# TaliMotzkin/GroupNet

Measured on AMD Instinct MI355X. Metric: scenes/sec GroupNet MS-HGNN forward, NBA N=11 B=512, 1/2/4/8 MI355X, higher is better.
Workload: dtype f32; 1 GPU; MS-HGNN forward (c2): affinity + top-k + pairwise + hyper scales [2, 5, 11], N=11 agents, 512 scenes per GPU (global batch 512), fp32 in and out (matrix stages: f16x3 — v_mfma_f32_32x32x16_f16, x = xh + xl (two fp16 parts), three part-products per product (fp32-accurate; operands beyond the fp16 range fall back to bf16x6 inside the launch)), device Philox noise, hipGraph replay on 4 alternating st; global_batch=512, agents=11, parallelism=batch-sharded x1

## Files before the change

groupnet_amd/csrc/gn_common.hpp:

```cpp
#pragma once
#include <hip/hip_runtime.h>
#include <stdint.h>
#include <stdlib.h>

#include "../../include/groupnet_hip.h"

#define GN_WAVE 64

typedef float f32x16 __attribute__((ext_vector_type(16)));
typedef float f32x4 __attribute__((ext_vector_type(4)));

static inline bool gn_aligned16(const void* p) { return (reinterpret_cast<uintptr_t>(p) & 15u) == 0; }

static inline int gn_check_launch() { return hipGetLastError() == hipSuccess ? GN_OK : GN_ERR_LAUNCH; }

#define GN_REQUIRE_PTR(p) \
  do {                    \
    if ((p) == nullptr) return GN_ERR_NULL; \
  } while (0)
#define GN_REQUIRE_ALIGNED(p) \
  do {                        \
    if (!gn_aligned16(p)) return GN_ERR_ALIGN; \
  } while (0)

__device__ __forceinline__ int gn_uniform(int v) { return __builtin_amdgcn_readfirstlane(v); }
template <typename T>
__device__ __forceinline__ T gn_uniform_load(const T* p) {
  return *(const __attribute__((address_space(4))) T*)p;
}

__device__ __forceinline__ float gn_half_sum(float v) {
#pragma unroll
  for (int m = 16; m >= 1; m >>= 1) v += __shfl_xor(v, m, GN_WAVE);
  return v;
}
__device__ __forceinline__ float gn_wave_sum(float v) {
#pragma unroll
  for (int m = 32; m >= 1; m >>= 1) v += __shfl_xor(v, m, GN_WAVE);
  return v;
}
__device__ __forceinline__ float gn_wave_max(float v) {
#pragma unroll
  for (int m = 32; m >= 1; m >>= 1) v = fmaxf(v, __shfl_xor(v, m, GN_WAVE));
  return v;
}

__device__ __forceinline__ float gn_nonmember_sum(int others, float mx) {
  return others > 0 ? (float)others * expf(0.f - mx) : 0.f;
}

template <typename K>
static inline void gn_allow_big_lds(K kernel) {
  static bool done = false;
  if (!done) {
    (void)hipFuncSetAttribute(reinterpret_cast<const void*>(kernel), hipFuncAttributeMaxDynamicSharedMemorySize,
                              160 * 1024);
    done = true;
  }
}

__device__ __forceinline__ void gn_philox_block(unsigned long long blk, unsigned long long seed, uint32_t (&c)[4]) {
  c[0] = (uint32_t)blk;
  c[1] = (uint32_t)(blk >> 32);
  c[2] = 0u;
  c[3] = 0u;
  uint32_t k0 = (uint32_t)seed, k1 = (uint32_t)(seed >> 32);
#pragma unroll
  for (int r = 0; r < 10; ++r) {
    const uint64_t p0 = (uint64_t)0xD2511F53u * c[0];
    const uint64_t p1 = (uint64_t)0xCD9E8D57u * c[2];
    const uint32_t n0 = (uint32_t)(p1 >> 32) ^ c[1] ^ k0;
    const uint32_t n1 = (uint32_t)p1;
    const uint32_t n2 = (uint32_t)(p0 >> 32) ^ c[3] ^ k1;
    const uint32_t n3 = (uint32_t)p0;
    c[0] = n0;
    c[1] = n1;
    c[2] = n2;
    c[3] = n3;
    k0 += 0x9E3779B9u;
    k1 += 0xBB67AE85u;
  }
}
__device__ __forceinline__ float gn_philox_to_uniform(uint32_t x) { return (float)(x >> 8) * 5.9604644775390625e-08f; }
__device__ __forceinline__ float gn_philox_uniform_at(unsigned long long idx, unsigned long long seed) {
  uint32_t c[4];
  gn_philox_block(idx >> 2, seed, c);
  const int l = (int)(idx & 3);
  const uint32_t x = l == 0 ? c[0] : (l == 1 ? c[1] : (l == 2 ? c[2] : c[3]));
  return gn_philox_to_uniform(x);
}

struct GnSwitches {
  bool xcd;
  bool pool_stage;
  bool agg_lines;
  bool agg_hstage;
  bool scatter_pairs;
  int edge_rb2, agg_rb2;
  int mlp2_xs;
  int n2e_rows;
  long long rb2_min_pairs;
};
static inline GnSwitches gn_read_switches() {
  auto tri = [](const char* name) {
    const char* e = getenv(name);
    return e == nullptr ? -1 : (atoi(e) != 0 ? 1 : 0);
  };
  GnSwitches sw{};
  sw.xcd = tri("GN_XCD") != 0;
  sw.pool_stage = tri("GN_POOL_STAGE") != 0;
  sw.agg_lines = tri("GN_AGG_LINES") != 0;
  sw.agg_hstage = tri("GN_AGG_HSTAGE") != 0;
  sw.scatter_pairs = tri("GN_SCATTER_PAIRS") != 0;
  sw.edge_rb2 = tri("GN_EDGE_RB2");
  sw.agg_rb2 = tri("GN_AGG_RB2");
  sw.mlp2_xs = tri("GN_MLP2_XS");
  sw.n2e_rows = tri("GN_N2E_ROWS");
  const char* e = getenv("GN_RB2_MIN_PAIRS");
  sw.rb2_min_pairs = e != nullptr && atoll(e) > 0 ? atoll(e) : 0;
  return sw;
}

static inline void plan_begin(gn_launch_plan_t& p, int n_groups) {
  p = gn_launch_plan_t{};
  p.n_groups = n_groups;
  p.grid[1] = p.grid[2] = 1;
}

#define GN_MAX_SECTIONS 32
struct XcdSections {
  int first[GN_MAX_SECTIONS + 1];
  int n;
  int enabled;
};
__device__ __forceinline__ int gn_xcd_logical(const XcdSections& S, int p) {
  if (!S.enabled) return p;
  const int x = p & 7;
  int slot = p >> 3;
  for (int g = 0; g < S.n; ++g) {
    const int W = S.first[g + 1] - S.first[g];
    const int lo = (int)(((long long)W * x) >> 3), hi = (int)(((long long)W * (x + 1)) >> 3);
    if (slot < hi - lo) return S.first[g] + lo + slot;
    slot -= hi - lo;
  }
  return -1;
}
static inline int gn_xcd_grid(XcdSections& S, bool on) {
  const int total = S.first[S.n];
  S.enabled = (on && S.n <= GN_MAX_SECTIONS && total >= 64) ? 1 : 0;
  if (!S.enabled) return total;
  int worst = 0;
  for (int x = 0; x < 8; ++x) {
    int c = 0;
    for (int g = 0; g < S.n; ++g) {
      const int W = S.first[g + 1] - S.first[g];
      c += (int)(((long long)W * (x + 1)) >> 3) - (int)(((long long)W * x) >> 3);
    }
    worst = c > worst ? c : worst;
  }
  return 8 * worst;
}

__host__ __device__ __forceinline__ int gn_pair_count(int N) { return N * (N + 1) / 2; }
__device__ __forceinline__ int gn_pair_start(int i, int N) { return i * N - (i * (i - 1)) / 2; }
__device__ __forceinline__ int gn_pair_index(int a, int b, int N) {
  const int i = a < b ? a : b, j = a < b ? b : a;
  return gn_pair_start(i, N) + (j - i);
}
__device__ __forceinline__ void gn_pair_decode(int p, int N, int& i, int& j) {
  const float t = (float)(2 * N + 1);
  int r = (int)((t - sqrtf(t * t - 8.f * (float)p)) * 0.5f);
  r = r < 0 ? 0 : (r > N - 1 ? N - 1 : r);
  while (r + 1 < N && gn_pair_start(r + 1, N) <= p) ++r;
  while (r > 0 && gn_pair_start(r, N) > p) --r;
  i = r;
  j = r + (p - gn_pair_start(r, N));
}
```

groupnet_amd/csrc/gn_mlp_bf16.hpp:

```cpp
#pragma once
#include "gn_mlp_common.hpp"
#include "gn_affinity.hpp"

#include <type_traits>

namespace {

constexpr int kOccP1 = 2;
template <int P>
constexpr int kNodeOcc = P == 2 ? 3 : 2;
template <int P>
constexpr int kEdgeOcc = P == 1 ? kOccP1 : (P == 2 ? 3 : 2);

template <int P>
struct Parts {
  bf16x8 p[P];
};

typedef float f32x8 __attribute__((ext_vector_type(8)));
__device__ __forceinline__ bf16x8 cvt_half(const f32x16& v, int hf) {
  f32x8 h;
#pragma unroll
  for (int jj = 0; jj < 8; ++jj) h[jj] = v[8 * hf + jj];
  return __builtin_convertvector(h, bf16x8);
}

typedef _Float16 f16x8 __attribute__((ext_vector_type(8)));
typedef _Float16 f16x2 __attribute__((ext_vector_type(2)));
typedef float f32x2 __attribute__((ext_vector_type(2)));
constexpr float kF16Limit = 65000.f;
struct ovf_t {
  unsigned long long mask;
  int wf;
};
template <int P>
__device__ __forceinline__ void make_parts(const f32x16& v, int hf, Parts<P>& x, ovf_t& ovf) {
  if constexpr (P == 3) {
#pragma unroll
    for (int jj = 0; jj < 8; ++jj) {
      __bf16 a, b, c;
      split3(v[8 * hf + jj], a, b, c);
      x.p[0][jj] = a;
      x.p[1][jj] = b;
      x.p[2][jj] = c;
    }
  }
  if constexpr (P == 2) {
    f16x8 hi, lo;
    float m[4];
#pragma unroll
    for (int j = 0; j < 4; ++j) {
      const float a = v[8 * hf + 2 * j], b = v[8 * hf + 2 * j + 1];
      m[j] = __builtin_fmaxf(__builtin_fabsf(a), __builtin_fabsf(b));
      const f32x2 pr = {a, b};
      const f16x2 hh = __builtin_convertvector(pr, f16x2);
      const f32x2 rem = {a - (float)hh[0], b - (float)hh[1]};
      const f16x2 ll = __builtin_convertvector(rem, f16x2);
      hi[2 * j] = hh[0], hi[2 * j + 1] = hh[1];
      lo[2 * j] = ll[0], lo[2 * j + 1] = ll[1];
    }
    x.p[0] = __builtin_bit_cast(bf16x8, hi);
    x.p[1] = __builtin_bit_cast(bf16x8, lo);
    ovf.mask |= __builtin_amdgcn_ballot_w64(__builtin_fmaxf(__builtin_fmaxf(m[0], m[1]), __builtin_fmaxf(m[2], m[3])) > kF16Limit);
  }
  if constexpr (P == 1) x.p[0] = cvt_half(v, hf);
}
typedef short i16x2 __attribute__((ext_vector_type(2)));
typedef __bf16 bf16x2 __attribute__((ext_vector_type(2)));
typedef unsigned u32x4 __attribute__((ext_vector_type(4)));
__device__ __forceinline__ void make_parts_relu(const f32x16& v, int hf, Parts<1>& x) {
  u32x4 r;
#pragma unroll
  for (int j = 0; j < 4; ++j) {
    const f32x2 pr = {v[8 * hf + 2 * j], v[8 * hf + 2 * j + 1]};
    const i16x2 zero = {0, 0};
    r[j] = __builtin_bit_cast(unsigned,
                              __builtin_elementwise_max(__builtin_bit_cast(i16x2, __builtin_convertvector(pr, bf16x2)), zero));
  }
  x.p[0] = __builtin_bit_cast(bf16x8, r);
}

template <int P, int NT>
__device__ __forceinline__ void make_parts_tiles(const f32x16 (&v)[NT], Parts<P> (&x)[NT][2], ovf_t& ovf) {
#pragma unroll
  for (int t = 0; t < NT; ++t) {
    make_parts<P>(v[t], 0, x[t][0], ovf);
    make_parts<P>(v[t], 1, x[t][1], ovf);
  }
}
template <int P>
constexpr int kMfmaPerSub = P == 3 ? 6 : (P == 2 ? 3 : 1);

template <int P, typename F>
__device__ __forceinline__ void run_with_fallback(F body) {
  ovf_t ovf = {0ull, 0};
  if constexpr (P == 2) {
    body(std::integral_constant<int, 2>{}, ovf);
    if (!__syncthreads_or(ovf.mask != 0ull || ovf.wf != 0)) return;
    ovf = {0ull, 0};
    body(std::integral_constant<int, 3>{}, ovf);
  } else {
    body(std::integral_constant<int, P>{}, ovf);
  }
}
__device__ __forceinline__ int image_flag(const void* image, int substeps) {
  return gn_uniform_load(reinterpret_cast<const int*>(reinterpret_cast<const char*>(image) + (size_t)substeps * 2 * 1024));
}
template <int P>
__device__ __forceinline__ const void* pick_image(const void* x, const void* h) { return P == 2 ? h : x; }

template <int P>
__device__ __forceinline__ void mfma_substep(const f32x4 (&w)[P], const Parts<P>& x, f32x16& acc) {
  if constexpr (P == 3) {
    const bf16x8 w1 = __builtin_bit_cast(bf16x8, w[0]);
    const bf16x8 w2 = __builtin_bit_cast(bf16x8, w[1]);
    const bf16x8 w3 = __builtin_bit_cast(bf16x8, w[2]);
    acc = __builtin_amdgcn_mfma_f32_32x32x16_bf16(w3, x.p[0], acc, 0, 0, 0);
    acc = __builtin_amdgcn_mfma_f32_32x32x16_bf16(w2, x.p[1], acc, 0, 0, 0);
    acc = __builtin_amdgcn_mfma_f32_32x32x16_bf16(w1, x.p[2], acc, 0, 0, 0);
    acc = __builtin_amdgcn_mfma_f32_32x32x16_bf16(w2, x.p[0], acc, 0, 0, 0);
    acc = __builtin_amdgcn_mfma_f32_32x32x16_bf16(w1, x.p[1], acc, 0, 0, 0);
    acc = __builtin_amdgcn_mfma_f32_32x32x16_bf16(w1, x.p[0], acc, 0, 0, 0);
  } else if constexpr (P == 2) {
    const f16x8 wh = __builtin_bit_cast(f16x8, w[0]), wl = __builtin_bit_cast(f16x8, w[1]);
    const f16x8 xh = __builtin_bit_cast(f16x8, x.p[0]), xl = __builtin_bit_cast(f16x8, x.p[1]);
    acc = __builtin_amdgcn_mfma_f32_32x32x16_f16(wh, xl, acc, 0, 0, 0);
    acc = __builtin_amdgcn_mfma_f32_32x32x16_f16(wl, xh, acc, 0, 0, 0);
    acc = __builtin_amdgcn_mfma_f32_32x32x16_f16(wh, xh, acc, 0, 0, 0);
  } else {
    acc = __builtin_amdgcn_mfma_f32_32x32x16_bf16(__builtin_bit_cast(bf16x8, w[0]), x.p[0], acc, 0, 0, 0);
  }
}

template <int P>
struct XStream {
  static constexpr int D = P == 1 ? 8 : 4;
  static constexpr int CH = 1;
  f32x4 q[D][P];
  const f32x4* cur;
  const f32x4* nxt;
  int seg;
  __device__ __forceinline__ void begin(const f32x4* first) {
#pragma unroll
    for (int u = 0; u < D; ++u)
#pragma unroll
      for (int p = 0; p < P; ++p) q[u][p] = first[(u * P + p) * 64];
  }
  __device__ __forceinline__ void segment(const f32x4* cur_, const f32x4* nxt_, int seg_) { cur = cur_, nxt = nxt_, seg = seg_; }
  template <bool FENCE = true>
  __device__ __forceinline__ void step(int, int s, const Parts<P>& x, f32x16& acc) {
    const int u = s % D;
    mfma_substep<P>(q[u], x, acc);
    const f32x4* src = s + D < seg ? cur + (size_t)(s + D) * P * 64 : nxt + (size_t)(s + D - seg) * P * 64;
#pragma unroll
    for (int p = 0; p < P; ++p) q[u][p] = src[p * 64];
    if constexpr (FENCE) __builtin_amdgcn_sched_barrier(0);
  }
};

template <int P, int LOOK_ = (P == 1 ? 4 : 2), int QD_ = (P == 1 ? 4 : 2)>
struct WStream {
  static constexpr int CH = P == 1 ? 8 : 4;
  static constexpr int LOOK = LOOK_;
  static constexpr int R = 3;
  static constexpr int PIECES = CH * P;
  static constexpr int PW = PIECES / 4;
  static constexpr int kChunkF4 = PIECES * 64;
  static constexpr int kRingF4 = R * kChunkF4;
  static constexpr int QD = QD_;
  const f32x4* rd_cur;
  const f32x4* rd_next;
  f32x4* wr;
  f32x4* ring0;
  const f32x4* ld;
  const f32x4* ld_last;
  int slot;
  f32x4 st[LOOK][PW];
  f32x4 q[QD][P];

  __device__ __forceinline__ static void barrier_drain() { asm volatile("s_waitcnt lgkmcnt(0)\n\ts_barrier" ::: "memory"); }
  __device__ __forceinline__ static void barrier() { asm volatile("s_barrier" ::: "memory"); }
// ... 351 lines not shown
  const float f1 = h == 0 ? b2k[32 + (lane & 31)] : 0.f;
  const float efb = h == 0 ? efk : 0.f;
  out[0] = __builtin_amdgcn_mfma_f32_32x32x2f32(f0, efb, out[0], 0, 0, 0);
  out[1] = __builtin_amdgcn_mfma_f32_32x32x2f32(f1, efb, out[1], 0, 0, 0);
}

__device__ __forceinline__ void add_b2_regs(float f0, float f1, float efk, int h, f32x16 (&out)[2]) {
  const float efb = h == 0 ? efk : 0.f;
  out[0] = __builtin_amdgcn_mfma_f32_32x32x2f32(h == 0 ? f0 : 0.f, efb, out[0], 0, 0, 0);
  out[1] = __builtin_amdgcn_mfma_f32_32x32x2f32(h == 0 ? f1 : 0.f, efb, out[1], 0, 0, 0);
}
constexpr int kAggPartBytes = 4 * 32 * (64 + 8) * 4;


template <int P, int L, int D_ = (P == 1 ? 8 : 4)>
struct PStream {
  static constexpr int D = D_;
  f32x4 q[D][P];
  template <typename AT>
  __device__ __forceinline__ void begin(AT at) {
#pragma unroll
    for (int u = 0; u < D; ++u)
      if (u < L) {
        const f32x4* src = at(u);
#pragma unroll
        for (int p = 0; p < P; ++p) q[u][p] = src[p * 64];
      }
  }
  template <typename AT>
  __device__ __forceinline__ void step(int s, AT at, const Parts<P>& x, f32x16& acc) {
    mfma_substep<P>(q[s % D], x, acc);
    if (s + D < L) {
      const f32x4* src = at(s + D);
#pragma unroll
      for (int p = 0; p < P; ++p) q[s % D][p] = src[p * 64];
    }
    __builtin_amdgcn_sched_barrier(0);
  }
};


template <int P>
__device__ __forceinline__ void put_parts(f32x4* lds, int tile, int lane, const f32x16& v, ovf_t& ovf) {
#pragma unroll
  for (int hf = 0; hf < 2; ++hf) {
    Parts<P> x;
    make_parts<P>(v, hf, x, ovf);
#pragma unroll
    for (int p = 0; p < P; ++p) lds[((tile * 2 + hf) * P + p) * 64 + lane] = __builtin_bit_cast(f32x4, x.p[p]);
  }
}
template <int P, int IT>
__device__ __forceinline__ void get_parts(const f32x4* lds, int lane, Parts<P> (&xi)[IT][2]) {
#pragma unroll
  for (int t = 0; t < IT; ++t)
#pragma unroll
    for (int hf = 0; hf < 2; ++hf)
#pragma unroll
      for (int p = 0; p < P; ++p) xi[t][hf].p[p] = __builtin_bit_cast(bf16x8, lds[((t * 2 + hf) * P + p) * 64 + lane]);
}
template <int OT>
__device__ __forceinline__ void put_partial(f32x4* lds, int wave, int lane, const f32x16 (&out)[OT]) {
#pragma unroll
  for (int q = 0; q < 4 * OT; ++q) {
    const f32x4 v = {out[q >> 2][4 * (q & 3) + 0], out[q >> 2][4 * (q & 3) + 1], out[q >> 2][4 * (q & 3) + 2],
                     out[q >> 2][4 * (q & 3) + 3]};
    lds[(wave * 4 * OT + q) * 64 + lane] = v;
  }
}
template <int OT>
__device__ __forceinline__ f32x4 sum_partial(const f32x4* lds, int q, int lane) {
  f32x4 v = lds[(0 * 4 * OT + q) * 64 + lane];
#pragma unroll
  for (int w = 1; w < 4; ++w) {
    const f32x4 a = lds[(w * 4 * OT + q) * 64 + lane];
    v[0] += a[0];
    v[1] += a[1];
    v[2] += a[2];
    v[3] += a[3];
  }
  return v;
}

__device__ __forceinline__ int pipe_off_A(int t, int NA, int NB) { return t == 0 ? 0 : NA + (t - 1) * (NA + NB); }
__device__ __forceinline__ int pipe_off_B(int t, int HT, int NA, int NB) {
  return t < HT - 1 ? 2 * NA + t * (NA + NB) : HT * NA + (HT - 1) * NB;
}

constexpr int kXPitch = 128 + 4;
template <int P>
struct ClosingStream {
  const f32x4* segA;
  const f32x4* segB;
  static constexpr int kDepth = 4;
  PStream<P, 12, kDepth> ps;
  __device__ __forceinline__ void init(const void* image, int wave, int lane, ovf_t& ovf) {
    if constexpr (P == 2) ovf.wf |= image_flag(image, 48);
    const f32x4* img = reinterpret_cast<const f32x4*>(image) + lane;
    segA = img + (size_t)pipe_off_A(wave, 8, 4) * P * 64;
    segB = img + (size_t)pipe_off_B(wave, 4, 8, 4) * P * 64;
  }
  __device__ __forceinline__ const f32x4* at(int s) const { return s < 8 ? segA + s * P * 64 : segB + (s - 8) * P * 64; }
  __device__ __forceinline__ void begin() {
    ps.begin([&](int s) { return at(s); });
  }
  __device__ __forceinline__ void step(int s, const Parts<P>& x, f32x16& acc) {
    ps.step(s, [&](int t) { return at(t); }, x, acc);
  }
};
template <int P, typename T>
__device__ __forceinline__ void closing_chain(ClosingStream<P>& cs, const float* __restrict__ bias, T* __restrict__ y, int ldy,
                                              int dout, int row0, int nlive, const float* __restrict__ X, f32x4* lds,
                                              int wave, int lane, ovf_t& ovf) {
  constexpr int IT = 4, HT = 4, OT = 2, NA = 2 * IT, NB = 2 * OT;
  const int h = lane >> 5, r = lane & 31;
  {
    f32x16 in;
    const float* xr = X + r * kXPitch + 32 * wave + 4 * h;
#pragma unroll
    for (int q = 0; q < 4; ++q) {
      const f32x4 v = *reinterpret_cast<const f32x4*>(xr + 8 * q);
      in[4 * q + 0] = v[0], in[4 * q + 1] = v[1], in[4 * q + 2] = v[2], in[4 * q + 3] = v[3];
    }
    put_parts<P>(lds, wave, lane, in, ovf);
  }
  __syncthreads();
  auto xop = [&](int u, Parts<P>& x) {
#pragma unroll
    for (int p = 0; p < P; ++p) x.p[p] = __builtin_bit_cast(bf16x8, lds[(u * P + p) * 64 + lane]);
  };
  Parts<P> xa[2];
  xop(0, xa[0]);
  const f32x16 bt = load_bias_tile(bias + 32 * wave, h);
  f32x16 hid;
#pragma unroll
  for (int q = 0; q < 16; ++q) hid[q] = 0.f;
#pragma unroll
  for (int u = 0; u < NA; ++u) {
    if (u + 1 < NA) xop(u + 1, xa[(u + 1) & 1]);
    cs.step(u, xa[u & 1], hid);
  }
  f32x16 out[OT], bo[OT];
#pragma unroll
  for (int o = 0; o < OT; ++o) {
    if (wave == 0) bo[o] = load_bias_tile(bias + 32 * HT + 32 * o, h);
#pragma unroll
    for (int q = 0; q < 16; ++q) out[o][q] = 0.f;
  }
#pragma unroll
  for (int q = 0; q < 16; ++q) hid[q] += bt[q];
  relu16(hid);
  Parts<P> xh[2];
  make_parts<P>(hid, 0, xh[0], ovf);
  make_parts<P>(hid, 1, xh[1], ovf);
#pragma unroll
  for (int u = 0; u < NB; ++u) cs.step(NA + u, xh[u & 1], out[u >> 1]);
  if (wave == 0) {
#pragma unroll
    for (int o = 0; o < OT; ++o)
#pragma unroll
      for (int q = 0; q < 16; ++q) out[o][q] += bo[o][q];
  }
  __syncthreads();
  put_partial<OT>(lds, wave, lane, out);
  __syncthreads();
  if (r < nlive) {
// ... 1301 lines not shown
#pragma unroll
  for (int r = 0; r < 16; ++r) acc[r] = 0.f;
  const T* fb = reinterpret_cast<const T*>(G.feat) + (size_t)b * E * GN_FEAT + 32 * tile;
  for (int j = 0; j < N; ++j) {
    add_row_tile(fb + (size_t)(n * N + j) * GN_FEAT, 1.f, h, acc);
    add_row_tile(fb + (size_t)(j * N + n) * GN_FEAT, 1.f, h, acc);
  }
#pragma unroll
  for (int r = 0; r < 16; ++r) in[r] = acc[r] / divisor;
}

constexpr int kLinePitch = 36;
template <typename T, bool hyper, int NRG>
__device__ __forceinline__ void scatter_tile_lines_(const gn_mlp2_group_t& G, int blk, int rows, int N, float divisor,
                                                    int tile, int lane, int rg0, float* __restrict__ scratch) {
  const int E = G.E;
  const int sub = lane >> 3, piece = lane & 7;
  const int cnt = hyper ? E : N;
  unsigned fo[NRG], ho[NRG];
  int nn[NRG];
#pragma unroll
  for (int rg = 0; rg < NRG; ++rg) {
    const int r = min(blk * 32 + (rg0 + rg) * 8 + sub, rows - 1);
    const int b = r / N;
    nn[rg] = r - b * N;
    fo[rg] = (unsigned)b * E * GN_FEAT + 32 * tile + 4 * piece;
    ho[rg] = (unsigned)b * E * N + nn[rg];
  }
  const T* feat = reinterpret_cast<const T*>(G.feat);
  f32x4 acc[NRG];
#pragma unroll
  for (int rg = 0; rg < NRG; ++rg) acc[rg] = f32x4{0.f, 0.f, 0.f, 0.f};
  constexpr int MB = NRG == 4 ? 6 : 11;
  for (int m0 = 0; m0 < cnt; m0 += MB) {
    f32x4 v[MB][NRG];
    float w[MB][hyper ? NRG : 1];
#pragma unroll
    for (int u = 0; u < MB; ++u) {
      const int m = min(m0 + u, cnt - 1);
#pragma unroll
      for (int rg = 0; rg < NRG; ++rg) {
        const int idx = hyper ? m : gn_pair_index(nn[rg], m, N);
        v[u][rg] = ld4(feat + fo[rg] + (size_t)idx * GN_FEAT);
        if constexpr (hyper) w[u][rg] = G.H[ho[rg] + (size_t)m * N];
      }
    }
#pragma unroll
    for (int u = 0; u < MB; ++u)
      if (m0 + u < cnt) {
#pragma unroll
        for (int rg = 0; rg < NRG; ++rg)
#pragma unroll
          for (int c = 0; c < 4; ++c) acc[rg][c] = fmaf(hyper ? w[u][hyper ? rg : 0] : 1.f, v[u][rg][c], acc[rg][c]);
      }
  }
#pragma unroll
  for (int rg = 0; rg < NRG; ++rg) {
    f32x4 o;
#pragma unroll
    for (int c = 0; c < 4; ++c) o[c] = acc[rg][c] / divisor;
    *reinterpret_cast<f32x4*>(scratch + ((rg0 + rg) * 8 + sub) * kLinePitch + 4 * piece) = o;
  }
}
template <typename T, int NRG = 4>
__device__ __forceinline__ bool scatter_tile_lines(const gn_mlp2_group_t& G, int blk, int rows, int N, float divisor,
                                                   int tile, int lane, float* __restrict__ scratch, int rg0 = 0) {
  if (G.H != nullptr) scatter_tile_lines_<T, true, NRG>(G, blk, rows, N, divisor, tile, lane, rg0, scratch);
  else if (G.sym) scatter_tile_lines_<T, false, NRG>(G, blk, rows, N, divisor, tile, lane, rg0, scratch);
  else return false;
  return true;
}
__device__ __forceinline__ void read_tile_lines(const float* __restrict__ scratch, int lane, f32x16& in) {
  const int j = lane & 31, h = lane >> 5;
#pragma unroll
  for (int q = 0; q < 4; ++q) {
    const f32x4 v = *reinterpret_cast<const f32x4*>(scratch + j * kLinePitch + 8 * q + 4 * h);
    in[4 * q + 0] = v[0];
    in[4 * q + 1] = v[1];
    in[4 * q + 2] = v[2];
    in[4 * q + 3] = v[3];
  }
}

template <int P, int IT, int OT>
constexpr int kXsLdsF4 = (IT * 2 * P * 64 > 4 * 4 * OT * 64) ? IT * 2 * P * 64 : 4 * 4 * OT * 64;
template <int P, typename T, int IT, int HT, int OT>
__device__ __forceinline__ void mlp2_xs_body(const GroupTable<gn_mlp2_group_t>& Tb, int rows, int dout, int ldy, int N,
                                             float divisor, f32x4* lds, float (*lines)[32 * kLinePitch], ovf_t& ovf) {
  static_assert(HT % 4 == 0, "hidden tiles are dealt over 4 waves");
  constexpr int TPW = HT / 4, NA = 2 * IT, NB = 2 * OT, L = TPW * (NA + NB);
  const int lwg = gn_uniform(gn_xcd_logical(Tb.xs, blockIdx.x));
  if (lwg < 0) return;
  const int gi = find_group(Tb, lwg);
  const gn_mlp2_group_t G = Tb.g[gi];
  const int wave = wave_id();
  const RowBlock rb = row_block(rows, lwg - Tb.first_wg[gi]);
  const int lane = rb.lane, h = rb.h;
  const float* b0 = G.bias;
  const float* b1 = G.bias + 32 * HT;
  const void* image = pick_image<P>(G.Wx, G.Wh);
  if constexpr (P == 2) ovf.wf |= image_flag(image, HT * (NA + NB));
  const f32x4* img = reinterpret_cast<const f32x4*>(image) + lane;
  const f32x4* segA[TPW];
  const f32x4* segB[TPW];
#pragma unroll
  for (int tt = 0; tt < TPW; ++tt) {
    const int t = wave + 4 * tt;
    segA[tt] = img + (size_t)pipe_off_A(t, NA, NB) * P * 64;
    segB[tt] = img + (size_t)pipe_off_B(t, HT, NA, NB) * P * 64;
  }
  auto at = [&](int s) -> const f32x4* {
    return s < TPW * NA ? segA[s / NA] + (s % NA) * P * 64 : segB[(s - TPW * NA) / NB] + ((s - TPW * NA) % NB) * P * 64;
  };
  PStream<P, L> ps;
  bool via_lines = false;
  f32x16 in;
  if constexpr (IT == 4) {
    if (G.x == nullptr) {
      via_lines = (G.H != nullptr || G.sym != 0) && G.E > 0;
      if (via_lines) {
        if (wave >= 2) mlp2_rows_tile<T>(G, rb.row_ld, h, N, divisor, IT, wave, in);
        scatter_tile_lines<T, 2>(G, lwg - Tb.first_wg[gi], rows, N, divisor, wave & 1, lane, lines[wave & 1], 2 * (wave >> 1));
        __syncthreads();
      }
    }
  }
  if (wave < IT) {
    if (via_lines && wave < 2) read_tile_lines(lines[wave], lane, in);
    else if (!(via_lines && wave >= 2)) mlp2_rows_tile<T>(G, rb.row_ld, h, N, divisor, IT, wave, in);
    ps.begin(at);
    if (G.in_out != nullptr && rb.live) store_tile(G.in_out + (size_t)rb.row * (32 * IT) + 32 * wave + 4 * h, in);
    put_parts<P>(lds, wave, lane, in, ovf);
  } else {
    ps.begin(at);
  }
  __syncthreads();
  auto xop = [&](int u, Parts<P>& x) {
#pragma unroll
    for (int p = 0; p < P; ++p) x.p[p] = __builtin_bit_cast(bf16x8, lds[(u * P + p) * 64 + lane]);
  };
  Parts<P> xa[2];
  xop(0, xa[0]);
  f32x16 hid[TPW], bt[TPW];
#pragma unroll
  for (int tt = 0; tt < TPW; ++tt) {
    bt[tt] = load_bias_tile(b0 + 32 * (wave + 4 * tt), h);
#pragma unroll
    for (int r = 0; r < 16; ++r) hid[tt][r] = 0.f;
  }
  int s = 0;
#pragma unroll
  for (int tt = 0; tt < TPW; ++tt)
#pragma unroll
    for (int u = 0; u < NA; ++u) {
      if (s + 1 < TPW * NA) xop((u + 1) % NA, xa[(s + 1) & 1]);
      ps.step(s, at, xa[s & 1], hid[tt]);
      ++s;
    }
  f32x16 out[OT], bo[OT];
#pragma unroll
  for (int o = 0; o < OT; ++o) {
    if (wave == 0) bo[o] = load_bias_tile(b1 + 32 * o, h);
#pragma unroll
    for (int r = 0; r < 16; ++r) out[o][r] = 0.f;
  }
#pragma unroll
  for (int tt = 0; tt < TPW; ++tt) {
#pragma unroll
    for (int r = 0; r < 16; ++r) hid[tt][r] += bt[tt][r];
    Parts<P> xh[2];
    if constexpr (P == 1) {
      make_parts_relu(hid[tt], 0, xh[0]);
      make_parts_relu(hid[tt], 1, xh[1]);
    } else {
      relu16(hid[tt]);
      if (G.hid_out != nullptr && rb.live)
        store_tile(G.hid_out + (size_t)rb.row * (32 * HT) + 32 * (wave + 4 * tt) + 4 * h, hid[tt]);
      make_parts<P>(hid[tt], 0, xh[0], ovf);
      make_parts<P>(hid[tt], 1, xh[1], ovf);
    }
#pragma unroll
    for (int u = 0; u < NB; ++u) {
      ps.step(s, at, xh[u & 1], out[u >> 1]);
      ++s;
    }
  }
  if (wave == 0) {
#pragma unroll
    for (int o = 0; o < OT; ++o)
#pragma unroll
      for (int r = 0; r < 16; ++r) out[o][r] += bo[o][r];
  }
  __syncthreads();
  put_partial<OT>(lds, wave, lane, out);
  __syncthreads();
  if (!rb.live) return;
  T* yrow = reinterpret_cast<T*>(G.y) + (size_t)rb.row * ldy;
  const bool vec = ((dout | ldy) & 3) == 0;
#pragma unroll
  for (int qq = 0; qq < OT; ++qq) {
    const int q = wave * OT + qq;
    const f32x4 v = sum_partial<OT>(lds, q, lane);
    const int f = 32 * (q >> 2) + 8 * (q & 3) + 4 * h;
    if (vec) {
      if (f < dout) st4(yrow + f, v);
    } else {
#pragma unroll
      for (int c = 0; c < 4; ++c)
        if (f + c < dout) st1(yrow + f + c, v[c]);
    }
  }
}
template <int P, typename T, int IT, int HT, int OT>
__global__ __launch_bounds__(256, HT == 4 ? 3 : 2) void mlp2_xs_kernel(GroupTable<gn_mlp2_group_t> Tb, int rows, int dout, int ldy, int N,
                                                          float divisor) {
  __shared__ f32x4 lds[kXsLdsF4<P == 2 ? 3 : P, IT, OT>];
  __shared__ __align__(16) float lines[2][32 * kLinePitch];
  run_with_fallback<P>([&](auto pc, ovf_t& ovf) {
    mlp2_xs_body<decltype(pc)::value, T, IT, HT, OT>(Tb, rows, dout, ldy, N, divisor, lds, lines, ovf);
  });
}

}
```

groupnet_amd/csrc/gn_mlp_mfma.hip:

```cpp
#include <stdlib.h>

#include <type_traits>

#include "gn_mlp_common.hpp"
#include "gn_mlp_bf16.hpp"

namespace {


__global__ void pack_linear_kernel(const float* __restrict__ W, float* __restrict__ Wp, int out_f, int in_f,
                                   int ld, int col_off, int OT, int IT) {
  const size_t total = (size_t)OT * IT * kTileFloats;
  for (size_t idx = (size_t)blockIdx.x * blockDim.x + threadIdx.x; idx < total;
       idx += (size_t)gridDim.x * blockDim.x) {
    const int c = idx & 3;
    const int lane = (idx >> 2) & 63;
    const int q = (idx >> 8) & 3;
    const size_t tile = idx >> 10;
    const int t = (int)(tile % IT), o = (int)(tile / IT);
    const int row = 32 * o + (lane & 31);
    const int col = 32 * t + 8 * q + 4 * (lane >> 5) + c;
    Wp[idx] = (row < out_f && col < in_f) ? W[(size_t)row * ld + col_off + col] : 0.f;
  }
}
// ... 1257 lines not shown
}
static int agg_entry(const gn_agg_group_t* groups, int n_groups, bool twin, gn_stream_t stream, gn_launch_plan_t* plan) {
  gn_launch_plan_t p;
  int order[GN_MAX_GROUPS], n = 0;
  GN_CHECK(agg_plan(groups, n_groups, twin, gn_read_switches(), plan != nullptr ? *plan : p, order, n));
  return plan != nullptr ? GN_OK : agg_launch(p, order, n, groups, (hipStream_t)stream);
}
extern "C" int gn_agg_mlp_f32(const gn_agg_group_t* groups, int n_groups, gn_stream_t stream) {
  return agg_entry(groups, n_groups, false, stream, nullptr);
}
extern "C" int gn_agg_mlp_bf16(const gn_agg_group_t* groups, int n_groups, gn_stream_t stream) {
  return agg_entry(groups, n_groups, true, stream, nullptr);
}
extern "C" int gn_agg_mlp_plan_f32(const gn_agg_group_t* groups, int n_groups, gn_launch_plan_t* plan) {
  GN_REQUIRE_PTR(plan);
  return agg_entry(groups, n_groups, false, nullptr, plan);
}
extern "C" int gn_agg_mlp_plan_bf16(const gn_agg_group_t* groups, int n_groups, gn_launch_plan_t* plan) {
  GN_REQUIRE_PTR(plan);
  return agg_entry(groups, n_groups, true, nullptr, plan);
}

extern "C" int gn_node_linear_f32(const float* x, const float* W, const float* bias, float* y, int rows, int dout,
                                  gn_stream_t stream) {
  const void* ptrs[] = {x, W, bias, y};
  for (const void* p : ptrs) GN_CHECK(need(p, true));
  if (rows <= 0 || dout <= 0 || dout % 128 != 0) return GN_ERR_SHAPE;
  hipLaunchKernelGGL(node_linear_kernel, dim3((rows + 31) / 32), dim3(256), 0, (hipStream_t)stream, x, W, bias, y, rows,
                     dout / 32);
  return gn_check_launch();
}

static int mlp2_plan(const gn_mlp2_group_t* groups, int n_groups, int rows, int din, int dh, int dout, int ldy, int N,
                     float divisor, bool twin, const GnSwitches& sw, gn_launch_plan_t& p) {
  GN_CHECK(check_groups(groups, n_groups));
  if (rows <= 0 || dout <= 0 || ldy < dout) return GN_ERR_SHAPE;
  int xm = x_mode(groups, n_groups, [](const gn_mlp2_group_t& G) { return G.Wx != nullptr; });
  if (xm < 0) return GN_ERR_SHAPE;
  if (twin && (xm != 1 || dout > 64)) return GN_ERR_SHAPE;
  if (xm == 1 && dout > 64) {
    xm = 0;
    for (int g = 0; g < n_groups; ++g)
      if (groups[g].W == nullptr) return GN_ERR_NULL;
  }
  plan_begin(p, n_groups);
  bool fused = false;
  bool wide_hyper = false;
  for (int g = 0; g < n_groups; ++g) {
    const gn_mlp2_group_t& G = groups[g];
    if (G.x != nullptr) {
      GN_CHECK(need(G.x, true));
    } else {
      if (din != 128 || N <= 0 || !(divisor != 0.f) || rows % N != 0 || G.E < 0) return GN_ERR_SHAPE;
      GN_CHECK(need(G.feat, true));
      GN_CHECK(need(G.ori, true));
      if (G.E > 0) {
        if (G.H == nullptr && G.E != (G.sym ? gn_pair_count(N) : N * N)) return GN_ERR_SHAPE;
        if (G.H != nullptr && G.sym) return GN_ERR_SHAPE;
      } else if (G.H != nullptr || G.sym) return GN_ERR_SHAPE;
    }
    GN_CHECK(need(xm ? G.Wx : (const void*)G.W, true));
    GN_CHECK(need(G.bias, true));
    GN_CHECK(need(G.y, false));
    if (twin && (G.in_out != nullptr || G.hid_out != nullptr)) return GN_ERR_SHAPE;
    fused = fused || G.x == nullptr || G.in_out != nullptr || G.hid_out != nullptr;
    wide_hyper = wide_hyper || (G.x == nullptr && G.H != nullptr && G.E > 16);
    p.pos[g] = g;
  }
  const bool widths_ok = (din == 64 || din == 128) && (dh == 128 || dh == 256);
  p.tiles[0] = din / 32;
  p.tiles[1] = dh / 32;
  const int blocks32 = (rows + 31) / 32;
  if (xm) {
    if (!twin) {
      const int hm = x_mode(groups, n_groups, [](const gn_mlp2_group_t& G) { return G.Wh != nullptr; });
      if (hm < 0) return GN_ERR_SHAPE;
      p.precision = hm ? 2 : 3;
    } else
      p.precision = 1;
    if (!widths_ok) return GN_ERR_SHAPE;
    p.tiles[2] = dout <= 32 ? 1 : 2;
    const bool xs = (sw.mlp2_xs >= 0 ? sw.mlp2_xs != 0 : (long long)blocks32 * n_groups <= 1536) && !wide_hyper;
    p.kernel = xs ? GN_K_MLP2_XS : GN_K_MLP2_X;
    for (int g = 0; g < n_groups; ++g) p.wgs[g] = xs ? blocks32 : row_grid(rows);
    plan_grid(p, n_groups, nullptr, true, sw);
    return GN_OK;
  }
  const bool use_split = dh == 128 && dout <= 64 && (long long)blocks32 * n_groups <= 1024 && (din == 64 || din == 128) &&
                         !fused;
  if (!use_split && !widths_ok) return GN_ERR_SHAPE;
  p.kernel = use_split ? GN_K_MLP2_SPLIT : GN_K_MLP2;
  p.grid[0] = use_split ? blocks32 : row_grid(rows);
  p.grid[1] = n_groups;
  for (int g = 0; g < n_groups; ++g) p.wgs[g] = p.grid[0];
  return GN_OK;
}
template <int P, typename T, typename F>
static int mlp2_x_dispatch(const gn_launch_plan_t& p, F&& f) {
  const bool xs = p.kernel == GN_K_MLP2_XS;
#define GN_MLP2_CASE(IT, HT, OT) \
  case IT * 100 + HT * 10 + OT: return xs ? f(mlp2_xs_kernel<P, T, IT, HT, OT>) : f(mlp2_x_kernel<P, T, IT, HT, OT>)
  switch (p.tiles[0] * 100 + p.tiles[1] * 10 + p.tiles[2]) {
    GN_MLP2_CASE(2, 4, 1);
    GN_MLP2_CASE(2, 4, 2);
    GN_MLP2_CASE(4, 4, 1);
    GN_MLP2_CASE(4, 4, 2);
    GN_MLP2_CASE(2, 8, 1);
    GN_MLP2_CASE(2, 8, 2);
    GN_MLP2_CASE(4, 8, 1);
    GN_MLP2_CASE(4, 8, 2);
  }
#undef GN_MLP2_CASE
  return GN_ERR_SHAPE;
}
template <typename F>
static int mlp2_dispatch(const gn_launch_plan_t& p, F&& f) {
  if (p.precision == 1) return mlp2_x_dispatch<1, __bf16>(p, f);
  if (p.precision == 2) return mlp2_x_dispatch<2, float>(p, f);
  if (p.precision == 3) return mlp2_x_dispatch<3, float>(p, f);
  if (p.kernel == GN_K_MLP2_SPLIT) return p.tiles[0] == 2 ? f(mlp2_split_kernel<2>) : f(mlp2_split_kernel<4>);
  if (p.tiles[0] == 2) return p.tiles[1] == 4 ? f(mlp2_kernel<2, 4>) : f(mlp2_kernel<2, 8>);
  return p.tiles[1] == 4 ? f(mlp2_kernel<4, 4>) : f(mlp2_kernel<4, 8>);
}
static int mlp2_launch(const gn_launch_plan_t& p, const gn_mlp2_group_t* groups, int rows, int dout, int ldy, int N,
                       float divisor, hipStream_t s) {
  GroupTable<gn_mlp2_group_t> T{};
  T.n = p.n_groups;
  for (int g = 0; g < T.n; ++g) T.g[g] = groups[g];
  if (p.precision != 0) {
    table_first_wg(T, p, nullptr);
    table_xcd_grid(T, p.xcd != 0);
  }
  return mlp2_dispatch(p, [&](auto k) {
    hipLaunchKernelGGL(k, dim3(p.grid[0], p.grid[1]), dim3(256), 0, s, T, rows, dout, ldy, N, divisor);
    return gn_check_launch();
  });
}
static int mlp2_entry(const gn_mlp2_group_t* groups, int n_groups, int rows, int din, int dh, int dout, int ldy, int N,
                      float divisor, bool twin, gn_stream_t stream, gn_launch_plan_t* plan) {
  gn_launch_plan_t p;
  GN_CHECK(mlp2_plan(groups, n_groups, rows, din, dh, dout, ldy, N, divisor, twin, gn_read_switches(), plan != nullptr ? *plan : p));
  return plan != nullptr ? GN_OK : mlp2_launch(p, groups, rows, dout, ldy, N, divisor, (hipStream_t)stream);
}
extern "C" int gn_mlp2_f32(const gn_mlp2_group_t* groups, int n_groups, int rows, int din, int dh, int dout, int ldy,
                           int N, float divisor, gn_stream_t stream) {
  return mlp2_entry(groups, n_groups, rows, din, dh, dout, ldy, N, divisor, false, stream, nullptr);
}
extern "C" int gn_mlp2_bf16(const gn_mlp2_group_t* groups, int n_groups, int rows, int din, int dh, int dout, int ldy,
                            int N, float divisor, gn_stream_t stream) {
  return mlp2_entry(groups, n_groups, rows, din, dh, dout, ldy, N, divisor, true, stream, nullptr);
}
extern "C" int gn_mlp2_plan_f32(const gn_mlp2_group_t* groups, int n_groups, int rows, int din, int dh, int dout, int ldy,
                                int N, float divisor, gn_launch_plan_t* plan) {
  GN_REQUIRE_PTR(plan);
  return mlp2_entry(groups, n_groups, rows, din, dh, dout, ldy, N, divisor, false, nullptr, plan);
}
extern "C" int gn_mlp2_plan_bf16(const gn_mlp2_group_t* groups, int n_groups, int rows, int din, int dh, int dout, int ldy,
                                 int N, float divisor, gn_launch_plan_t* plan) {
  GN_REQUIRE_PTR(plan);
  return mlp2_entry(groups, n_groups, rows, din, dh, dout, ldy, N, divisor, true, nullptr, plan);
}
```

Measured before the change: 7.477 million scenes/s.

## Stage hyperedge features and incidence in LDS for MLP2 xs scatter path

Adds an optional staged path in the mlp2_xs kernel: for hyper groups, the features and H incidence covering a 32-row block are copied into LDS once and the node gather is computed from LDS, replacing the line-based scatter. It also merges the separate lines buffer into the shared LDS region, sized as the max of operands, partials and lines. The final reduction now keeps each wave's own partial in registers, writing only the other waves' quads to LDS. The fallback OR now goes through an explicit LDS-word reduction. Staging is gated on GN_MLP2_STAGE, which defaults to on, and on fit within the region; it adds extra syncs and LDS traffic per block.

```diff
diff --git a/groupnet_amd/csrc/gn_common.hpp b/groupnet_amd/csrc/gn_common.hpp
--- a/groupnet_amd/csrc/gn_common.hpp
+++ b/groupnet_amd/csrc/gn_common.hpp
@@ -95,6 +95,7 @@
   bool pool_stage;
   bool agg_lines;
   bool agg_hstage;
+  bool mlp2_stage;
   bool scatter_pairs;
   int edge_rb2, agg_rb2;
   int mlp2_xs;
@@ -111,6 +112,7 @@
   sw.pool_stage = tri("GN_POOL_STAGE") != 0;
   sw.agg_lines = tri("GN_AGG_LINES") != 0;
   sw.agg_hstage = tri("GN_AGG_HSTAGE") != 0;
+  sw.mlp2_stage = tri("GN_MLP2_STAGE") != 0;
   sw.scatter_pairs = tri("GN_SCATTER_PAIRS") != 0;
   sw.edge_rb2 = tri("GN_EDGE_RB2");
   sw.agg_rb2 = tri("GN_AGG_RB2");
diff --git a/groupnet_amd/csrc/gn_mlp_bf16.hpp b/groupnet_amd/csrc/gn_mlp_bf16.hpp
--- a/groupnet_amd/csrc/gn_mlp_bf16.hpp
+++ b/groupnet_amd/csrc/gn_mlp_bf16.hpp
@@ -97,6 +97,28 @@
   if constexpr (P == 2) {
     body(std::integral_constant<int, 2>{}, ovf);
     if (!__syncthreads_or(ovf.mask != 0ull || ovf.wf != 0)) return;
+    ovf = {0ull, 0};
+    body(std::integral_constant<int, 3>{}, ovf);
+  } else {
+    body(std::integral_constant<int, P>{}, ovf);
+  }
+}
+__device__ __forceinline__ bool workgroup_or(int* words, bool flag) {
+  __syncthreads();
+  const int any = __any(flag);
+  if ((threadIdx.x & 63) == 0) words[threadIdx.x >> 6] = any;
+  __syncthreads();
+  int r = 0;
+  for (int w = 0; w < (int)(blockDim.x >> 6); ++w) r |= words[w];
+  return r != 0;
+}
+template <int P, typename F>
+__device__ __forceinline__ void run_with_fallback(F body, int* words) {
+  ovf_t ovf = {0ull, 0};
+  if constexpr (P == 2) {
+    body(std::integral_constant<int, 2>{}, ovf);
+    if (!workgroup_or(words, ovf.mask != 0ull || ovf.wf != 0)) return;
+    __syncthreads();
     ovf = {0ull, 0};
     body(std::integral_constant<int, 3>{}, ovf);
   } else {
@@ -614,6 +636,42 @@
   return v;
 }
 
+template <typename F>
+__device__ __forceinline__ void for_wave(int wave, F f) {
+  switch (wave) {
+    case 0: f(std::integral_constant<int, 0>{}); break;
+    case 1: f(std::integral_constant<int, 1>{}); break;
+    case 2: f(std::integral_constant<int, 2>{}); break;
+    default: f(std::integral_constant<int, 3>{}); break;
+  }
+}
+template <int OT>
+__device__ __forceinline__ f32x4 out_quad(const f32x16 (&out)[OT], int q) {
+  return f32x4{out[q >> 2][4 * (q & 3) + 0], out[q >> 2][4 * (q & 3) + 1], out[q >> 2][4 * (q & 3) + 2],
+               out[q >> 2][4 * (q & 3) + 3]};
+}
+constexpr int partial_slot(int w, int q, int OT) { return w * 3 * OT + (q < w * OT ? q : q - OT); }
+template <int OT, int W>
+__device__ __forceinline__ void put_partial_others(f32x4* lds, int lane, const f32x16 (&out)[OT]) {
+#pragma unroll
+  for (int q = 0; q < 4 * OT; ++q)
+    if (q / OT != W) lds[partial_slot(W, q, OT) * 64 + lane] = out_quad<OT>(out, q);
+}
+template <int OT, int W>
+__device__ __forceinline__ f32x4 sum_partial_own(const f32x4* lds, int qq, int lane, const f32x16 (&out)[OT]) {
+  const int q = W * OT + qq;
+  f32x4 v = W == 0 ? out_quad<OT>(out, q) : lds[partial_slot(0, q, OT) * 64 + lane];
+#pragma unroll
+  for (int w = 1; w < 4; ++w) {
+    const f32x4 a = w == W ? out_quad<OT>(out, q) : lds[partial_slot(w, q, OT) * 64 + lane];
+    v[0] += a[0];
+    v[1] += a[1];
+    v[2] += a[2];
+    v[3] += a[3];
+  }
+  return v;
+}
+
 __device__ __forceinline__ int pipe_off_A(int t, int NA, int NB) { return t == 0 ? 0 : NA + (t - 1) * (NA + NB); }
 __device__ __forceinline__ int pipe_off_B(int t, int HT, int NA, int NB) {
   return t < HT - 1 ? 2 * NA + t * (NA + NB) : HT * NA + (HT - 1) * NB;
@@ -2081,11 +2139,68 @@
   }
 }
 
-template <int P, int IT, int OT>
-constexpr int kXsLdsF4 = (IT * 2 * P * 64 > 4 * 4 * OT * 64) ? IT * 2 * P * 64 : 4 * 4 * OT * 64;
+__host__ __device__ inline int mlp2_stage_scenes(int N) { return 31 / N + 2; }
+template <typename T>
+__host__ __device__ inline size_t mlp2_stage_bytes(int N, int E) {
+  return (size_t)mlp2_stage_scenes(N) * E * (PoolStage<T>::kPitch * sizeof(T) + (size_t)N * sizeof(float));
+}
+template <typename T>
+__device__ __forceinline__ int mlp2_stage_fill(const gn_mlp2_group_t& G, int blk, int rows, int N, T* __restrict__ s_feat,
+                                               float*& s_H) {
+  using PS = PoolStage<T>;
+  const int E = G.E;
+  const int b0 = (blk * 32) / N, b1 = min(rows - 1, blk * 32 + 31) / N;
+  const int nrows = (b1 - b0 + 1) * E;
+  const T* src = reinterpret_cast<const T*>(G.feat) + (size_t)b0 * E * GN_FEAT;
+  for (int idx = threadIdx.x; idx < nrows * PS::kRowPieces; idx += blockDim.x) {
+    const int r = idx / PS::kRowPieces, c = idx - r * PS::kRowPieces;
+    *reinterpret_cast<f32x4*>(s_feat + r * PS::kPitch + c * PS::kPiece) =
+        *reinterpret_cast<const f32x4*>(src + (size_t)idx * PS::kPiece);
+  }
+  s_H = reinterpret_cast<float*>(s_feat + nrows * PS::kPitch);
+  const float* Hs = G.H + (size_t)b0 * E * N;
+  for (int idx = threadIdx.x; idx < nrows * N; idx += blockDim.x) s_H[idx] = Hs[idx];
+  return b0;
+}
+template <typename T>
+__device__ __forceinline__ void scatter_tile_staged(const T* __restrict__ s_feat, const float* __restrict__ s_H, int b0,
+                                                    int row, int N, int E, float divisor, int tile, int h, f32x16& in) {
+  using PS = PoolStage<T>;
+  constexpr int MB = 4;
+  const int b = row / N, n = row - b * N;
+  const T* fb = s_feat + (b - b0) * E * PS::kPitch + 32 * tile;
+  const float* hc = s_H + (b - b0) * E * N + n;
+  f32x16 acc;
+#pragma unroll
+  for (int r = 0; r < 16; ++r) acc[r] = 0.f;
+  for (int e0 = 0; e0 < E; e0 += MB) {
+    f32x16 v[MB];
+    float w[MB];
+#pragma unroll
+    for (int u = 0; u < MB; ++u) {
+      const int e = min(e0 + u, E - 1);
+      w[u] = hc[e * N];
+      load_row_tile(fb + e * PS::kPitch, h, v[u]);
+    }
+#pragma unroll
+    for (int u = 0; u < MB; ++u)
+      if (e0 + u < E) {
+#pragma unroll
+        for (int r = 0; r < 16; ++r) acc[r] = fmaf(w[u], v[u][r], acc[r]);
+      }
+  }
+#pragma unroll
+  for (int r = 0; r < 16; ++r) in[r] = acc[r] / divisor;
+}
+
+constexpr size_t xs_region_bytes(int parts, int IT, int OT) {
+  const int P = parts == 2 ? 3 : parts;
+  const int operands = IT * 2 * P * 64, partial = 4 * 3 * OT * 64, lines = IT == 4 ? 2 * 32 * kLinePitch / 4 : 0;
+  return sizeof(f32x4) * (operands > partial ? (operands > lines ? operands : lines) : (partial > lines ? partial : lines));
+}
 template <int P, typename T, int IT, int HT, int OT>
 __device__ __forceinline__ void mlp2_xs_body(const GroupTable<gn_mlp2_group_t>& Tb, int rows, int dout, int ldy, int N,
-                                             float divisor, f32x4* lds, float (*lines)[32 * kLinePitch], ovf_t& ovf) {
+                                             float divisor, unsigned staged_groups, f32x4* lds, ovf_t& ovf) {
   static_assert(HT % 4 == 0, "hidden tiles are dealt over 4 waves");
   constexpr int TPW = HT / 4, NA = 2 * IT, NB = 2 * OT, L = TPW * (NA + NB);
   const int lwg = gn_uniform(gn_xcd_logical(Tb.xs, blockIdx.x));
@@ -2112,26 +2227,38 @@
     return s < TPW * NA ? segA[s / NA] + (s % NA) * P * 64 : segB[(s - TPW * NA) / NB] + ((s - TPW * NA) % NB) * P * 64;
   };
   PStream<P, L> ps;
-  bool via_lines = false;
+  bool via_lds = false, begun = false;
   f32x16 in;
   if constexpr (IT == 4) {
     if (G.x == nullptr) {
-      via_lines = (G.H != nullptr || G.sym != 0) && G.E > 0;
-      if (via_lines) {
+      const bool staged = (staged_groups >> gi & 1u) != 0;
+      via_lds = staged || ((G.H != nullptr || G.sym != 0) && G.E > 0);
+      if (via_lds) {
         if (wave >= 2) mlp2_rows_tile<T>(G, rb.row_ld, h, N, divisor, IT, wave, in);
-        scatter_tile_lines<T, 2>(G, lwg - Tb.first_wg[gi], rows, N, divisor, wave & 1, lane, lines[wave & 1], 2 * (wave >> 1));
+        if (staged) {
+          ps.begin(at);
+          begun = true;
+          float* s_H;
+          const int b0 = mlp2_stage_fill<T>(G, lwg - Tb.first_wg[gi], rows, N, reinterpret_cast<T*>(lds), s_H);
+          __syncthreads();
+          if (wave < 2) scatter_tile_staged<T>(reinterpret_cast<const T*>(lds), s_H, b0, rb.row_ld, N, G.E, divisor, wave, h, in);
+        } else {
+          float* lines = reinterpret_cast<float*>(lds) + (wave & 1) * 32 * kLinePitch;
+          scatter_tile_lines<T, 2>(G, lwg - Tb.first_wg[gi], rows, N, divisor, wave & 1, lane, lines, 2 * (wave >> 1));
+          __syncthreads();
+          if (wave < 2) read_tile_lines(lines, lane, in);
+        }
         __syncthreads();
       }
     }
   }
   if (wave < IT) {
-    if (via_lines && wave < 2) read_tile_lines(lines[wave], lane, in);
-    else if (!(via_lines && wave >= 2)) mlp2_rows_tile<T>(G, rb.row_ld, h, N, divisor, IT, wave, in);
-    ps.begin(at);
+    if (!via_lds) mlp2_rows_tile<T>(G, rb.row_ld, h, N, divisor, IT, wave, in);
+    if (!begun) ps.begin(at);
     if (G.in_out != nullptr && rb.live) store_tile(G.in_out + (size_t)rb.row * (32 * IT) + 32 * wave + 4 * h, in);
     put_parts<P>(lds, wave, lane, in, ovf);
   } else {
-    ps.begin(at);
+    if (!begun) ps.begin(at);
   }
   __syncthreads();
   auto xop = [&](int u, Parts<P>& x) {
@@ -2191,33 +2318,36 @@
       for (int r = 0; r < 16; ++r) out[o][r] += bo[o][r];
   }
   __syncthreads();
-  put_partial<OT>(lds, wave, lane, out);
+  for_wave(wave, [&](auto w) { put_partial_others<OT, decltype(w)::value>(lds, lane, out); });
   __syncthreads();
   if (!rb.live) return;
   T* yrow = reinterpret_cast<T*>(G.y) + (size_t)rb.row * ldy;
   const bool vec = ((dout | ldy) & 3) == 0;
-#pragma unroll
-  for (int qq = 0; qq < OT; ++qq) {
-    const int q = wave * OT + qq;
-    const f32x4 v = sum_partial<OT>(lds, q, lane);
-    const int f = 32 * (q >> 2) + 8 * (q & 3) + 4 * h;
-    if (vec) {
-      if (f < dout) st4(yrow + f, v);
-    } else {
-#pragma unroll
-      for (int c = 0; c < 4; ++c)
-        if (f + c < dout) st1(yrow + f + c, v[c]);
-    }
-  }
+  for_wave(wave, [&](auto w) {
+    constexpr int W = decltype(w)::value;
+#pragma unroll
+    for (int qq = 0; qq < OT; ++qq) {
+      constexpr int q0 = W * OT;
+      const int q = q0 + qq;
+      const f32x4 v = sum_partial_own<OT, W>(lds, qq, lane, out);
+      const int f = 32 * (q >> 2) + 8 * (q & 3) + 4 * h;
+      if (vec) {
+        if (f < dout) st4(yrow + f, v);
+      } else {
+#pragma unroll
+        for (int c = 0; c < 4; ++c)
+          if (f + c < dout) st1(yrow + f + c, v[c]);
+      }
+    }
+  });
 }
 template <int P, typename T, int IT, int HT, int OT>
 __global__ __launch_bounds__(256, HT == 4 ? 3 : 2) void mlp2_xs_kernel(GroupTable<gn_mlp2_group_t> Tb, int rows, int dout, int ldy, int N,
-                                                          float divisor) {
-  __shared__ f32x4 lds[kXsLdsF4<P == 2 ? 3 : P, IT, OT>];
-  __shared__ __align__(16) float lines[2][32 * kLinePitch];
+                                                          float divisor, unsigned staged_groups) {
+  __shared__ f32x4 lds[xs_region_bytes(P, IT, OT) / sizeof(f32x4)];
   run_with_fallback<P>([&](auto pc, ovf_t& ovf) {
-    mlp2_xs_body<decltype(pc)::value, T, IT, HT, OT>(Tb, rows, dout, ldy, N, divisor, lds, lines, ovf);
-  });
-}
-
-}
+    mlp2_xs_body<decltype(pc)::value, T, IT, HT, OT>(Tb, rows, dout, ldy, N, divisor, staged_groups, lds, ovf);
+  }, reinterpret_cast<int*>(lds));
+}
+
+}
diff --git a/groupnet_amd/csrc/gn_mlp_mfma.hip b/groupnet_amd/csrc/gn_mlp_mfma.hip
--- a/groupnet_amd/csrc/gn_mlp_mfma.hip
+++ b/groupnet_amd/csrc/gn_mlp_mfma.hip
@@ -1363,6 +1363,12 @@
     p.tiles[2] = dout <= 32 ? 1 : 2;
     const bool xs = (sw.mlp2_xs >= 0 ? sw.mlp2_xs != 0 : (long long)blocks32 * n_groups <= 1536) && !wide_hyper;
     p.kernel = xs ? GN_K_MLP2_XS : GN_K_MLP2_X;
+    const size_t region = xs_region_bytes(p.precision, p.tiles[0], p.tiles[2]);
+    for (int g = 0; g < n_groups; ++g) {
+      const gn_mlp2_group_t& G = groups[g];
+      const bool hyper = xs && sw.mlp2_stage && G.x == nullptr && G.H != nullptr && G.E > 0 && N <= 16;
+      p.stage[g] = hyper && (twin ? mlp2_stage_bytes<__bf16>(N, G.E) : mlp2_stage_bytes<float>(N, G.E)) <= region;
+    }
     for (int g = 0; g < n_groups; ++g) p.wgs[g] = xs ? blocks32 : row_grid(rows);
     plan_grid(p, n_groups, nullptr, true, sw);
     return GN_OK;
@@ -1380,7 +1386,8 @@
 static int mlp2_x_dispatch(const gn_launch_plan_t& p, F&& f) {
   const bool xs = p.kernel == GN_K_MLP2_XS;
 #define GN_MLP2_CASE(IT, HT, OT) \
-  case IT * 100 + HT * 10 + OT: return xs ? f(mlp2_xs_kernel<P, T, IT, HT, OT>) : f(mlp2_x_kernel<P, T, IT, HT, OT>)
+  case IT * 100 + HT * 10 + OT: \
+    return xs ? f(mlp2_xs_kernel<P, T, IT, HT, OT>, std::true_type{}) : f(mlp2_x_kernel<P, T, IT, HT, OT>, std::false_type{})
   switch (p.tiles[0] * 100 + p.tiles[1] * 10 + p.tiles[2]) {
     GN_MLP2_CASE(2, 4, 1);
     GN_MLP2_CASE(2, 4, 2);
@@ -1399,9 +1406,10 @@
   if (p.precision == 1) return mlp2_x_dispatch<1, __bf16>(p, f);
   if (p.precision == 2) return mlp2_x_dispatch<2, float>(p, f);
   if (p.precision == 3) return mlp2_x_dispatch<3, float>(p, f);
-  if (p.kernel == GN_K_MLP2_SPLIT) return p.tiles[0] == 2 ? f(mlp2_split_kernel<2>) : f(mlp2_split_kernel<4>);
-  if (p.tiles[0] == 2) return p.tiles[1] == 4 ? f(mlp2_kernel<2, 4>) : f(mlp2_kernel<2, 8>);
-  return p.tiles[1] == 4 ? f(mlp2_kernel<4, 4>) : f(mlp2_kernel<4, 8>);
+  const std::false_type no{};
+  if (p.kernel == GN_K_MLP2_SPLIT) return p.tiles[0] == 2 ? f(mlp2_split_kernel<2>, no) : f(mlp2_split_kernel<4>, no);
+  if (p.tiles[0] == 2) return p.tiles[1] == 4 ? f(mlp2_kernel<2, 4>, no) : f(mlp2_kernel<2, 8>, no);
+  return p.tiles[1] == 4 ? f(mlp2_kernel<4, 4>, no) : f(mlp2_kernel<4, 8>, no);
 }
 static int mlp2_launch(const gn_launch_plan_t& p, const gn_mlp2_group_t* groups, int rows, int dout, int ldy, int N,
                        float divisor, hipStream_t s) {
@@ -1412,8 +1420,13 @@
     table_first_wg(T, p, nullptr);
     table_xcd_grid(T, p.xcd != 0);
   }
-  return mlp2_dispatch(p, [&](auto k) {
-    hipLaunchKernelGGL(k, dim3(p.grid[0], p.grid[1]), dim3(256), 0, s, T, rows, dout, ldy, N, divisor);
+  unsigned staged = 0;
+  for (int g = 0; g < T.n; ++g) staged |= p.stage[g] ? 1u << g : 0u;
+  return mlp2_dispatch(p, [&](auto k, auto xs) {
+    if constexpr (decltype(xs)::value)
+      hipLaunchKernelGGL(k, dim3(p.grid[0], p.grid[1]), dim3(256), 0, s, T, rows, dout, ldy, N, divisor, staged);
+    else
+      hipLaunchKernelGGL(k, dim3(p.grid[0], p.grid[1]), dim3(256), 0, s, T, rows, dout, ldy, N, divisor);
     return gn_check_launch();
   });
 }
```

Result: no change. 7.557 million scenes/s, median of 5 (+1.1%).
